# LeoQLi/DeepSIR

Measured on AMD Instinct MI355X. Metric: registered pairs/sec (5k-pt 3DMatch-shaped synthetic pairs, 5 registration iterations, KNN pyramid included), higher is better.
Workload: dtype f32 (GEMMs as fp16-pair MFMA, fp32 accumulate; index decisions exact fp32)

## Files before the change

deepsir_amd/_lib.py:

```python
from __future__ import annotations

import ctypes as C
import os

_HERE = os.path.dirname(os.path.abspath(__file__))
LIB_PATH = os.environ.get("DSIR_LIB", os.path.join(_HERE, "libdsir.so"))

c_float_p = C.POINTER(C.c_float)
c_i32_p = C.POINTER(C.c_int32)
c_i64_p = C.POINTER(C.c_int64)


class dsir_cfg(C.Structure):
    _fields_ = [
        ("feat_len", C.c_int32),
        ("num_knn", C.c_int32),
        ("num_layers", C.c_int32),
        ("sub_sampling_ratio", C.c_int32 * 4),
        ("d_out", C.c_int32 * 4),
        ("out_feat_dim", C.c_int32),
        ("num_classes", C.c_int32),
        ("max_points", C.c_int32),
        ("max_pairs", C.c_int32),
        ("pipeline", C.c_int32),
# ... 46 lines not shown
    "dsir_create_ex": (C.c_int, [C.c_int, C.POINTER(dsir_cfg), C.c_int, C.POINTER(C.c_void_p)]),
    "dsir_destroy": (None, [C.c_void_p]),
    "dsir_last_error": (C.c_char_p, [C.c_void_p]),
    "dsir_stream": (C.c_void_p, [C.c_void_p]),
    "dsir_sync": (C.c_int, [C.c_void_p]),
    "dsir_set_stream": (C.c_int, [C.c_void_p, C.c_void_p, C.c_int]),
    "dsir_num_weights": (C.c_int, [C.c_void_p]),
    "dsir_weight_name": (C.c_char_p, [C.c_void_p, C.c_int, c_i64_p]),
    "dsir_load_weight": (C.c_int, [C.c_void_p, C.c_char_p, C.c_void_p, c_i64_p, C.c_int]),
    "dsir_finalize_weights": (C.c_int, [C.c_void_p]),
    "dsir_narrow_i64": (C.c_int, [C.c_void_p, C.c_void_p, C.c_void_p, C.c_int64]),
    "dsir_knn_pyramid": (C.c_int, [C.c_void_p, C.c_void_p, C.c_int, C.c_int, C.c_int, C.c_void_p, C.c_void_p,
                                   C.c_void_p, C.c_void_p]),
    "dsir_randla_forward": (C.c_int, [C.c_void_p, C.c_int, C.c_void_p, C.c_int, C.c_int, C.c_int, C.c_void_p,
                                      C.c_void_p, C.c_void_p, C.c_void_p, C.c_void_p, C.c_void_p]),
    "dsir_ppf_pre": (C.c_int, [C.c_void_p, C.c_int, C.c_void_p, C.c_int, C.c_void_p, C.c_int64, C.c_int, C.c_int, C.c_void_p]),
    "dsir_estimate_normals": (C.c_int, [C.c_void_p, C.c_void_p, C.c_int, C.c_void_p, C.c_int64, C.c_int, C.c_int, c_float_p, C.c_void_p,
                                        C.c_void_p]),
    "dsir_estimate_normals_csr": (C.c_int, [C.c_void_p, C.c_void_p, C.c_int, C.c_void_p, C.c_void_p, C.c_int, C.c_int, c_float_p, C.c_void_p,
                                            C.c_void_p]),
    "dsir_fpfh": (C.c_int, [C.c_void_p, C.c_void_p, C.c_int, C.c_void_p, C.c_void_p, C.c_int64, C.c_void_p, C.c_void_p, C.c_int, C.c_int,
                            C.c_void_p, C.c_int, C.c_void_p]),
    "dsir_iss_keypoints": (C.c_int, [C.c_void_p, C.c_void_p, C.c_int, C.c_void_p, C.c_void_p, C.c_void_p, C.c_void_p, C.c_int, C.c_int,
                                     C.c_double, C.c_double, C.c_int, C.c_void_p, C.c_void_p, C.c_void_p, C.c_void_p]),
    "dsir_score": (C.c_int, [C.c_void_p, C.c_void_p, C.c_void_p, C.c_void_p, C.c_int64, C.c_void_p, C.c_int64,
                             C.c_int, C.c_int, C.c_void_p, C.c_void_p]),
    "dsir_aggregate": (C.c_int, [C.c_void_p, C.c_void_p, C.c_int64, C.c_void_p, C.c_void_p, C.c_int, C.c_int,
                                 C.c_void_p]),
    "dsir_nn_match": (C.c_int, [C.c_void_p, C.c_void_p, C.c_void_p, C.c_int, C.c_int, C.c_int, C.c_void_p]),
    "dsir_nn_match_screened": (C.c_int, [C.c_void_p, C.c_void_p, C.c_void_p, C.c_int, C.c_int, C.c_int, C.c_void_p, c_i64_p]),
# ... 189 lines not shown
```

deepsir_amd/csrc/att_pool.hip:

```cpp
#include "kernels.h"
#include "device_utils.h"
#include "att_pool_body.h"

namespace dsir {

namespace {

using namespace attp;

template <bool UV>
__global__ __launch_bounds__(256) __attribute__((amdgpu_waves_per_eu(UV ? 4 : 5, UV ? 4 : 5))) void att_pool16_kernel(const AttPool16Args p) {
  constexpr int LD = 20;
  constexpr int TB = 32 * LD + 32;
  __shared__ float s_sc[16];
  __shared__ float s_sh[16];
  __shared__ __attribute__((aligned(16))) float s_t[4][TB + 32 * LD];

  const int tid = threadIdx.x, lane = tid & 63, w = __builtin_amdgcn_readfirstlane(tid >> 6);
  const int m = lane & 31, h = lane >> 5;
  const int wi = xcd_contiguous(blockIdx.x, gridDim.x);
  const int bx = wi % p.grid_x;
  const int cloud = wi / p.grid_x;

  float sc[8], sh[8];
  const float slope = (h ? p.enc_act : p.f_act) ? 0.2f : 1.f;

  h8 whA, wlA, whB, wlB;
  {
    const _Float16* Wh = reinterpret_cast<const _Float16*>(p.Wh);
    const _Float16* Wl = reinterpret_cast<const _Float16*>(p.Wl);
    const int col = m & 15;
// ... 2 lines not shown
    h8 z;
#pragma unroll
    for (int j = 0; j < 8; ++j) z[j] = (_Float16)0.f;
    whA = m < 16 ? vh : z; wlA = m < 16 ? vl : z;
    whB = m < 16 ? z : vh; wlB = m < 16 ? z : vl;
  }
  const int pm = (m >> 2) & 1, km = ((m >> 3) << 2) | (m & 3);
  const float* fb = p.f + cloud * p.f_cs;
  const float* eb = p.enc + cloud * p.enc_cs;
  const int32_t* nbb = p.neigh + cloud * p.neigh_cs;
  float* Yb = p.Y + cloud * p.y_cs;
  float* T = &s_t[w][0];
  const int etile = m >> 4, ecol = m & 15;

  const int units = (p.n + 3) >> 2;
  const int nw = p.grid_x * 4;
  int u = bx * 4 + w;

  auto point_of = [&](int uu, int tile) { return min(4 * uu + 2 * tile + pm, p.n - 1); };
  auto load_idx = [&](int uu, int (&j)[2]) {
#pragma unroll
    for (int t = 0; t < 2; ++t) j[t] = nbb[(uint32_t)point_of(uu, t) * 16u + (uint32_t)km];
  };
  const float* uvb = UV ? p.uv + cloud * p.uv_cs : nullptr;
  const float* distb = UV ? p.dist + cloud * p.dist_cs : nullptr;
  float wa[8];
#pragma unroll
  for (int c = 0; c < 8; ++c) wa[c] = UV ? p.w8[c * 8] : 0.f;
  auto load_rows = [&](int uu, const int (&j)[2], float (&a)[2][8], float (&v)[2][8], float (&dd)[2]) {
#pragma unroll
    for (int t = 0; t < 2; ++t) {
      const int pt = point_of(uu, t);
// ... 72 lines not shown
    float mx = fmaxf(acc[0], acc[1]);
#pragma unroll
    for (int i = 2; i < 16; i += 2) mx = fmaxf(mx, fmaxf(acc[i], acc[i + 1]));
    const float ml = -mx * L2E;
    float se = 0.f, o = 0.f;
    const float* Tc = &T[etile * TB + 4 * h * LD + ecol];
#pragma unroll
    for (int i = 0; i < 16; ++i) {
      const float e = __builtin_amdgcn_exp2f(fmaf(acc[i], L2E, ml));
      const float x = Tc[(8 * (i >> 2) + (i & 3)) * LD];
      se += e;
      o = fmaf(x, e, o);
    }
    const int pt = 4 * u + 2 * etile + h;
    if (pt < p.n) Yb[(uint32_t)pt * 16u + (uint32_t)ecol] = o * __builtin_amdgcn_rcpf(se);
    __builtin_amdgcn_wave_barrier();
#pragma unroll
    for (int t = 0; t < 2; ++t) {
#pragma unroll
      for (int j = 0; j < 8; ++j) { a[t][j] = an[t][j]; av[t][j] = avn[t][j]; }
      ad[t] = adn[t];
    }
    u = un;
  }
}

template <int KH, bool UV>
__global__ __launch_bounds__(256) __attribute__((amdgpu_waves_per_eu(KH == 32 ? 3 : 2, KH == 32 ? 3 : 2))) void att_full_kernel(const AttPool16Args p) {
  constexpr int NCB = KH / 32;
  __shared__ __attribute__((aligned(16))) char smem[att_full_smem_bytes<KH>()];
  const int wi = xcd_contiguous(blockIdx.x, gridDim.x);
  att_full_body<KH, UV>(p, wi % p.grid_x, (wi / p.grid_x) % NCB, wi / (p.grid_x * NCB), smem);
}

__global__ __launch_bounds__(512) void att_full128_kernel(const AttPool16Args p) {
  constexpr int KH = 64, KC = 64, NS = 8, NT = 4;
  constexpr int LD = 72;
  __shared__ float s_sc[2 * KH];
// ... 125 lines not shown
          const float e = __builtin_amdgcn_exp2f(fmaf(acc[tt][i], L2E, ml));
          const float x = Tc[(8 * (i >> 2) + (i & 3)) * LD];
          se += e;
          o = fmaf(x, e, o);
        }
        if (pt < p.n) Yb[(uint32_t)pt * (uint32_t)(2 * KH) + (uint32_t)(64 * tp + 32 * tt + m)] = o * __builtin_amdgcn_rcpf(se);
      }
      __builtin_amdgcn_wave_barrier();
    }
    u = un;
  }
}

}

bool launch_att_pool16(const AttPool16Args& a, hipStream_t st) {
  if (a.n <= 0 || a.clouds <= 0) return true;
  if (!a.Wh || !a.Wl || !a.f || !a.neigh || !a.Y) return false;
  if (!a.enc && (!a.uv || !a.dist || !a.w8 || (reinterpret_cast<uintptr_t>(a.uv) % 16) != 0 || (a.uv_cs % 4) != 0)) return false;
  if ((a.ldw % 8) != 0 || (reinterpret_cast<uintptr_t>(a.Wh) % 16) != 0 || (reinterpret_cast<uintptr_t>(a.Wl) % 16) != 0) return false;
  if ((reinterpret_cast<uintptr_t>(a.f) % 16) != 0 || (a.f_cs % 4) != 0 || (a.f_ld % 4) != 0 || (a.enc && ((reinterpret_cast<uintptr_t>(a.enc) % 16) != 0 || (a.enc_cs % 4) != 0))) return false;
  if ((a.f_gn.stats && (8 % a.f_gn.groups) != 0) || (a.enc_gn.stats && (8 % a.enc_gn.groups) != 0)) return false;
  if ((int64_t)a.n * 16 * 8 * 4 >= ((int64_t)1 << 32)) return false;
  const int units = (a.n + 3) / 4;
  int blocks = (units + 31) / 32;
  const int64_t total = (int64_t)blocks * a.clouds;
  if (total < 512) {
    const int want = (int)((512 + (int64_t)a.clouds - 1) / (int64_t)a.clouds), most = (units + 3) / 4;
    const int nb = want < most ? want : most;
    if (nb > blocks) blocks = nb;
  }
  if (blocks < 1) blocks = 1;
  AttPool16Args b = a;
  b.grid_x = blocks;
  if (a.enc) hipLaunchKernelGGL(att_pool16_kernel<false>, dim3((unsigned)((int64_t)blocks * a.clouds)), dim3(256), 0, st, b);
  else hipLaunchKernelGGL(att_pool16_kernel<true>, dim3((unsigned)((int64_t)blocks * a.clouds)), dim3(256), 0, st, b);
  return true;
}

bool launch_att_full(const AttPool16Args& a, int KH, hipStream_t st) {
  if (a.n <= 0 || a.clouds <= 0) return true;
  if ((KH != 32 && KH != 64) || !a.Wh || !a.Wl || !a.f || !a.neigh || !a.Y) return false;
  if (!a.enc && (KH != 32 || !a.uv || !a.dist || !a.w8 || (reinterpret_cast<uintptr_t>(a.uv) % 16) != 0 || (a.uv_cs % 4) != 0)) return false;
  if ((a.ldw % 8) != 0 || (reinterpret_cast<uintptr_t>(a.Wh) % 16) != 0 || (reinterpret_cast<uintptr_t>(a.Wl) % 16) != 0) return false;
  if ((reinterpret_cast<uintptr_t>(a.f) % 16) != 0 || (a.f_cs % 4) != 0 || (a.f_ld % 4) != 0 || (a.enc && ((reinterpret_cast<uintptr_t>(a.enc) % 16) != 0 || (a.enc_cs % 4) != 0))) return false;
  if ((a.f_gn.stats && (KH % a.f_gn.groups) != 0) || (a.enc_gn.stats && (KH % a.enc_gn.groups) != 0)) return false;
  if ((int64_t)a.n * 16 * KH * 4 >= ((int64_t)1 << 32)) return false;
  const int units = (a.n + 1) / 2;
  if (KH == 64 && (int64_t)units * a.clouds >= 8192) {
    int blocks = (units + 63) / 64;
    if ((int64_t)blocks * a.clouds < 256) {
      const int want = (int)((256 + (int64_t)a.clouds - 1) / (int64_t)a.clouds), most = (units + 7) / 8;
      const int nb = want < most ? want : most;
      if (nb > blocks) blocks = nb;
    }
    if (blocks < 1) blocks = 1;
// ... 41 lines not shown
```

deepsir_amd/csrc/device_utils.h:

```cpp
#pragma once
#include <hip/hip_runtime.h>
#include <stdint.h>

namespace dsir {

typedef float f32x4 __attribute__((ext_vector_type(4)));

#ifndef DSIR_GN_WORDS_DEFINED
#define DSIR_GN_WORDS_DEFINED
constexpr int kGnWords = 4;
#endif

__device__ __forceinline__ float ld_f32(const float* base, uint32_t byte_off) {
  return *reinterpret_cast<const float*>(reinterpret_cast<const char*>(base) + byte_off);
}
__device__ __forceinline__ int ld_i32(const int32_t* base, uint32_t byte_off) {
  return *reinterpret_cast<const int32_t*>(reinterpret_cast<const char*>(base) + byte_off);
}
__device__ __forceinline__ void st_f32(float* base, uint32_t byte_off, float v) {
  *reinterpret_cast<float*>(reinterpret_cast<char*>(base) + byte_off) = v;
}

__device__ __forceinline__ int xcd_contiguous(int id, int nwg) {
  const int q8 = nwg >> 3, r8 = nwg & 7, xcd = id & 7;
// ... 62 lines not shown
  return v;
}

__device__ __forceinline__ float se3_row(const float* T, int r, float x, float y, float z) {
  return __fadd_rn(fmaf(z, T[r * 4 + 2], fmaf(y, T[r * 4 + 1], __fmul_rn(x, T[r * 4 + 0]))), T[r * 4 + 3]);
}

__device__ __forceinline__ float exp_neg(float x) {
  return __builtin_amdgcn_exp2f(x * 1.44269504088896340736f);
}

__device__ __forceinline__ double gn_stat_limb(double v, int limb) {
  const double l1 = rint(v * 0x1p-24);
  return limb ? rint(fma(-l1, 0x1p24, v) * 0x1p16) : l1;
}
__device__ __forceinline__ void gn_block_commit(const float* part, int n0, int ncols, int gw, double* stats_cloud) {
  const int g0 = n0 / gw, ng = (n0 + ncols - 1) / gw - g0 + 1;
  const int t = threadIdx.x, j = t & 15;
  for (int q = t >> 4; q < ((ng * 2 + 15) & ~15); q += 16) {
    const bool live = q < ng * 2;
    const int g = g0 + (q >> 1), stat = q & 1;
    const int c0 = max(g * gw, n0) - n0, c1 = min((g + 1) * gw, n0 + ncols) - n0;
    double d = 0.0;
    if (live)
      for (int c = c0 + j; c < c1; c += 16) d += (double)part[c * 2 + stat];
    d += __shfl_xor(d, 1); d += __shfl_xor(d, 2); d += __shfl_xor(d, 4); d += __shfl_xor(d, 8);
    if (live && j < 2)
      unsafeAtomicAdd(stats_cloud + (int64_t)g * kGnWords + 2 * stat + j, gn_stat_limb(d, j));
  }
}
__device__ __forceinline__ double gn_rstd(double var) {
  const double v = var + 1e-5;
  double r = __builtin_amdgcn_rsq(v);
  r = fma(r, fma(-0.5 * v * r, r, 0.5), r);
  r = fma(r, fma(-0.5 * v * r, r, 0.5), r);
  return r;
}
__device__ __forceinline__ double gn_stat_get(const double* slot) {
#ifdef DSIR_GN_STATS_COHERENT
  const double l1 = __hip_atomic_load(slot, __ATOMIC_RELAXED, __HIP_MEMORY_SCOPE_AGENT);
  const double l0 = __hip_atomic_load(slot + 1, __ATOMIC_RELAXED, __HIP_MEMORY_SCOPE_AGENT);
  return fma(l1, 0x1p24, l0 * 0x1p-16);
#else
  return fma(slot[0], 0x1p24, slot[1] * 0x1p-16);
// ... 64 lines not shown
```

deepsir_amd/csrc/engine_ctx.h:

```cpp
#pragma once
#include <hip/hip_runtime.h>

#include <string>
#include <unordered_map>
#include <vector>

#include "dsir.h"
#include "kernels.h"
#include "search_plan.h"

namespace dsir {

struct HostParam {
  std::string name;
  std::vector<int64_t> shape;
  std::vector<float> data;
  bool loaded = false;
  bool ignored = false;
  int64_t numel() const { int64_t n = 1; for (auto s : shape) n *= s; return n; }
};

struct Mlp2dW { const float *W = nullptr, *b = nullptr, *gamma = nullptr, *beta = nullptr; int cin = 0, cout = 0, groups = 0; };
struct AttW { const float* fc = nullptr; const float* fc_g = nullptr; int d = 0; Mlp2dW mlp; };
struct BlockW { Mlp2dW mlp1, lfa1, lfa2, mlp2, skip; AttW att1, att2; int d_in = 0, d = 0; const float* lse_w8 = nullptr;
// ... 183 lines not shown
  float* dist_buf[DSIR_MAX_LEVELS] = {};
  float* enc2_buf[DSIR_MAX_LEVELS] = {};
  double* enc_stats[DSIR_MAX_LEVELS] = {};
  double* enc2_stats[DSIR_MAX_LEVELS] = {};
  Act enc[DSIR_MAX_LEVELS], enc2[DSIR_MAX_LEVELS];
  static size_t stats_words(const dsir_cfg& g, int P) { return (size_t)2 * g.num_layers * gn_layer_words(P); }
  int plan(dsir_ctx* c, const Pyramid& ps, double* prezeroed);
};

struct AggExtras { float* sq = nullptr; void* hi = nullptr; void* lo = nullptr; unsigned long long* packed_init = nullptr; };

void fill_pyramid_layout(const dsir_cfg& cfg, int clouds, int n, Pyramid& p);
int gn_max_contributions(const dsir_cfg& g, int n, int flags = 0);
int randla_forward(dsir_ctx* c, const RandlaW& w, const Seg& in0, const Seg* in1, const Pyramid& py, float* feat_out,
                   float* logits_out, EncCache* cache = nullptr);
int run_ppf_pre(dsir_ctx* c, const RandlaW& w, const float* rows, int stride, const int32_t* neigh, int64_t neigh_cs, int clouds, int n,
                float* out);
float* run_mlp_feat(dsir_ctx* c, const float* feat0, int clouds, int n, float* out = nullptr);
bool run_att_proj(dsir_ctx* c, const float* xyz, int64_t xyz_cs, const float* score, const float* F, int clouds, int n,
                  float* desc, const AggExtras* ex = nullptr);
int build_pyramid(dsir_ctx* c, const float* points, int stride, int clouds, int n, float* xyz, int32_t* neigh,
                  int32_t* sub, int32_t* interp);

void expect_state_dict(dsir_ctx* c);

struct DescSearch {
  dsir_ctx* c;
  SearchMode mode;
  int P, J, K;
  bool timed = false;
// ... 33 lines not shown
```

deepsir_amd/csrc/entries_stage.hip:

```cpp
#include <cmath>

#include "engine_ctx.h"

using namespace dsir;

extern "C" {

int dsir_narrow_i64(dsir_ctx* c, const int64_t* src, int32_t* dst, int64_t n) {
  Call call(c); if (call.refused()) return 1;
  launch_narrow_i64(src, dst, n, c->stream);
  return call.finish();
}

int dsir_knn_pyramid(dsir_ctx* c, const float* points, int stride, int clouds, int n, float* xyz, int32_t* neigh,
                     int32_t* sub, int32_t* interp) {
  Call call(c); if (call.refused()) return 1;
  if (clouds < 1 || stride < 3) return fail(c, "dsir_knn_pyramid: bad arguments");
  if (int r = build_pyramid(c, points, stride, clouds, n, xyz, neigh, sub, interp)) return r;
  return call.finish();
}

int dsir_randla_forward(dsir_ctx* c, int which, const float* features, int cin, int clouds, int n, const float* xyz,
                        const int32_t* neigh, const int32_t* sub, const int32_t* interp, float* feat, float* logits) {
  Call call(c, Call::kWeights); if (call.refused()) return 1;
  if (which != 0 && c->cfg.pipeline != DSIR_PIPELINE_ALIGN) return fail(c, "randla_forward: this context has no inlier_model (pipeline != align)");
  const RandlaW& w = which == 0 ? c->net.feat : c->net.inl;
  if (w.ppf ? cin < 6 : cin != w.cin)
    return w.ppf ? fail(c, "randla_forward: use_ppf needs rows of xyz + normal, at least 6 columns, got %d (reference RandLANet.py:325)", cin)
                 : fail(c, "randla_forward: expected %d input channels, got %d", w.cin, cin);
  if (check_batch(c, "randla_forward", clouds, n)) return 1;
  Pyramid py;
  fill_pyramid_layout(c->cfg, clouds, n, py);
  if (py.nl[3] < kKnn) return fail(c, "cloud too small (n=%d)", n);
  py.xyz = xyz; py.neigh = neigh; py.sub = sub; py.interp = interp;
  const Seg in0 = plain_seg(features, (int64_t)n * cin, w.ppf ? 3 : cin, cin);
  const Seg in1 = plain_seg(features + 3, (int64_t)n * cin, 3, cin);
  if (int r = call.begin_walker()) return r;
  if (int r = randla_forward(c, w, in0, w.ppf ? &in1 : nullptr, py, feat, logits)) return r;
  return call.finish();
}

int dsir_ppf_pre(dsir_ctx* c, int which, const float* rows, int stride, const int32_t* neigh, int64_t neigh_cs, int clouds, int n,
                 float* out) {
  Call call(c, Call::kWeights); if (call.refused()) return 1;
  if (!(c->flags & DSIR_FLAG_PPF)) return fail(c, "dsir_ppf_pre: the context was not created with DSIR_FLAG_PPF");
  if (which != 0 && c->cfg.pipeline != DSIR_PIPELINE_ALIGN) return fail(c, "dsir_ppf_pre: this context has no inlier_model (pipeline != align)");
  if (!rows || !neigh || !out || clouds < 1 || n < kKnn) return fail(c, "dsir_ppf_pre: bad arguments");
  if (stride < 6) return fail(c, "dsir_ppf_pre: rows of xyz + normal need at least 6 columns, got %d (reference RandLANet.py:325)", stride);
  if (check_batch(c, "dsir_ppf_pre", clouds, n)) return 1;
  if (int r = run_ppf_pre(c, which == 0 ? c->net.feat : c->net.inl, rows, stride, neigh, neigh_cs, clouds, n, out)) return r;
  return call.finish();
}

// ... 128 lines not shown
```

deepsir_amd/csrc/kernels.h:

```cpp
#pragma once
#include <hip/hip_runtime.h>
#include <stdint.h>
#include <stdlib.h>

namespace dsir {

constexpr int kKnn = 16;

const char* tuning_env(const char* name);
inline bool tuning_flag(const char* name) { return tuning_env(name) != nullptr; }
inline long long tuning_int(const char* name, long long dflt) { const char* e = tuning_env(name); return e ? atoll(e) : dflt; }

#ifndef DSIR_GN_WORDS_DEFINED
#define DSIR_GN_WORDS_DEFINED
constexpr int kGnWords = 4;
#endif
struct GnRef {
  const double* stats;
  const float* gamma;
  const float* beta;
  int groups;
  double inv_count;
};

// ... 78 lines not shown
  const float* enc = nullptr;
  int64_t enc_cs = 0;
  const float* uv = nullptr; int64_t uv_cs = 0;
  const float* dist = nullptr; int64_t dist_cs = 0;
  const float* w8 = nullptr;
  GnRef enc_gn = {nullptr, nullptr, nullptr, 0, 0.0}; int enc_act = 1;
  const int32_t* neigh = nullptr;
  int64_t neigh_cs = 0;
  const void* Wh = nullptr;
  const void* Wl = nullptr;
  int ldw = 16;
  float* Y = nullptr;
  int64_t y_cs = 0;
  int n = 0, clouds = 0;
  int grid_x = 0;
};
bool launch_att_pool16(const AttPool16Args& a, hipStream_t st);
bool launch_att_full(const AttPool16Args& a, int KH, hipStream_t st);

struct LseUvArgs {
  const float* xyz = nullptr; int64_t xyz_cs = 0;
  const int32_t* neigh = nullptr; int64_t neigh_cs = 0;
  const float* w8 = nullptr;
  float* uv = nullptr; int64_t uv_cs = 0;
  float* dist = nullptr; int64_t dist_cs = 0;
  double* stats_out = nullptr; int groups = 0;
  int n = 0, clouds = 0, KH = 0;
  int vgrid = 0;
};
bool launch_lse_uv_stats(const LseUvArgs& a, hipStream_t st);

struct PpfArgs {
// ... 340 lines not shown
```

deepsir_amd/csrc/schedule.hip:

```cpp
#include <cstddef>
#include <cstring>
#include <vector>

#include "engine_ctx.h"

namespace dsir {

namespace {
void level_sizes(const dsir_cfg& cfg, int n, int* nl) {
  nl[0] = n;
  for (int l = 0; l < cfg.num_layers; ++l) nl[l + 1] = nl[l] / cfg.sub_sampling_ratio[l];
}
}

void fill_pyramid_layout(const dsir_cfg& cfg, int clouds, int n, Pyramid& p) {
  p.clouds = clouds; p.n = n;
  level_sizes(cfg, n, p.nl);
  p.off[0] = 0; p.soff[0] = 0;
  for (int l = 0; l < cfg.num_layers; ++l) { p.off[l + 1] = p.off[l] + p.nl[l]; p.soff[l + 1] = p.soff[l] + p.nl[l + 1]; }
  p.S = p.off[cfg.num_layers]; p.S1 = p.soff[cfg.num_layers];
}

int gn_max_contributions(const dsir_cfg& g, int n, int flags) {
  const bool ppf = (flags & DSIR_FLAG_PPF) != 0;
// ... 2 lines not shown
    const int groups = cout >= 64 ? 8 : 4;
    const int c = cin <= 64 ? pw_stream_gn_contributions(M, cout) : pw_tile_gn_contributions(M, cout, groups);
    if (c > worst) worst = c;
  };
  int nl[DSIR_MAX_LEVELS + 1];
  level_sizes(g, n, nl);
  const int L = g.num_layers;
  if (ppf) { const int c = ppf_gn_contributions(nl[0]); if (c > worst) worst = c; }
  else layer(nl[0], 6 > g.feat_len ? 6 : g.feat_len, 8);
  int dim = ppf ? 12 : 8;
  for (int l = 0; l < L; ++l) {
    const int d = g.d_out[l], m = nl[l], mk = nl[l] * kKnn;
    if (ppf && l == 0) { const int c = pw_gemm_gn_contributions(m); if (c > worst) worst = c; }
    else { layer(m, dim, d / 2); layer(m, dim, 2 * d); }
    if (d / 2 == 8 || d / 2 == 32) { const int c = lse_uv_gn_contributions(m, d / 2); if (c > worst) worst = c; }
    layer(mk, 10, d / 2);
    layer(mk, d / 2, d / 2);
    layer(m, d, d / 2); layer(m, d, d); layer(m, d, 2 * d);
    dim = 2 * d;
  }
  layer(nl[L], dim, dim);
  int dcur = dim;
  for (int j = 0; j < L; ++j) {
    const int lvl = L - 1 - j;
    const int cin = j < L - 1 ? dcur + 2 * g.d_out[L - j - 2] : 4 * g.d_out[0];
    dcur = j < L - 1 ? 2 * g.d_out[L - j - 2] : 2 * g.d_out[0];
    layer(nl[lvl], cin, dcur);
  }
  return worst;
}
// ... 177 lines not shown
    rec_flush();
    if (!c->ws.overflow && !launch_pw_gemm(a, st)) refuse("lfa.mlp1: no kernel took the relative-position layer");
    return y;
  }
  AttPool16Args att_pool_args(const AttW& w, const Act& f, const Act& enc, const int32_t* neigh, int64_t neigh_cs, int n, const Act& y) const {
    AttPool16Args a;
    a.f = f.p; a.f_cs = (int64_t)f.rows * f.C; a.f_ld = f.C; a.f_gn = f.gn; a.f_act = f.act;
    a.enc = enc.p; a.enc_cs = (int64_t)enc.rows * enc.C; a.enc_gn = enc.gn; a.enc_act = enc.act;
    a.uv = enc.uv; a.uv_cs = (int64_t)n * 2 * enc.C; a.dist = enc.dist; a.dist_cs = (int64_t)n * kKnn; a.w8 = enc.w8;
    a.neigh = neigh; a.neigh_cs = neigh_cs;
    const size_t off = (size_t)(w.fc - c->dweights);
    a.Wh = c->dweights16 + off; a.Wl = c->dweights16 + c->nweights + off; a.ldw = w.d;
    a.Y = y.p; a.y_cs = (int64_t)n * w.d; a.n = n; a.clouds = clouds;
    return a;
  }
  Act att(const AttW& w, const Act& f, const Act& enc, const int32_t* neigh, int64_t neigh_cs, int n, float* s2 = nullptr,
          int s2_mode = 0) {
    Act y;
    y.p = c->ws.get<float>((size_t)clouds * n * w.d);
    y.C = w.d; y.rows = n;
    const bool halves = f.C * 2 == w.d && enc.C * 2 == w.d;
    const bool fc16 = c->dweights16 && w.fc >= c->dweights && w.fc < c->dweights + c->nweights;
    if (w.d == 16 && halves && fc16) {
      const AttPool16Args a = att_pool_args(w, f, enc, neigh, neigh_cs, n, y);
      rec_flush();
      if (!c->ws.overflow && launch_att_pool16(a, st)) return y;
    } else if ((w.d == 64 || w.d == 128) && halves && fc16 && (enc.p || w.d == 64)) {
      const AttPool16Args a = att_pool_args(w, f, enc, neigh, neigh_cs, n, y);
      if (c->ws.overflow) return y;
      if (rec) {
        WalkJob j;
        if (walk_plan_att_full(a, w.d / 2, rec_wpc, &j) && rec_push(j)) return y;
        rec_flush();
      }
      if (launch_att_full(a, w.d / 2, st)) return y;
    } else if (att_keeps_score_cache(w.d) && w.fc_g && halves && enc.p) {
      float* G = c->ws.get<float>((size_t)clouds * n * w.d);
      GemmArgs g;
      g.amode = A_SEGS; g.nseg = 1; g.seg[0] = seg_of(f);
      g.W = w.fc_g; g.ldw = w.d / 2; g.bias = nullptr; g.Cin = w.d / 2; g.Cout = w.d; g.M = n; g.clouds = clouds;
// ... 93 lines not shown
  for (int l = 0; l < g.num_layers; ++l) {
    enc_stats[l] = cst + (size_t)(2 * l) * gn_layer_words(P);
    enc2_stats[l] = cst + (size_t)(2 * l + 1) * gn_layer_words(P);
  }
  return 0;
}

int run_ppf_pre(dsir_ctx* c, const RandlaW& w, const float* rows, int stride, const int32_t* neigh, int64_t neigh_cs, int clouds, int n,
                float* out) {
  const size_t stats_need = gn_layer_words(clouds, 4);
  if (stats_need > c->stats_cap) return fail(c, "stats arena too small (%zu > %zu)", stats_need, c->stats_cap);
  c->call.stats_top = 0;
  HIP_OK(c, hipMemsetAsync(c->stats, 0, stats_need * sizeof(double), c->stream));
  Sched s{c, c->stream, clouds};
  s.ppf_pre(w.pre, plain_seg(rows, (int64_t)n * stride, 3, stride), plain_seg(rows + 3, (int64_t)n * stride, 3, stride), neigh, neigh_cs, n, out);
  return 0;
}

int randla_forward(dsir_ctx* c, const RandlaW& w, const Seg& in0, const Seg* in1, const Pyramid& py, float* feat_out,
                   float* logits_out, EncCache* cache) {
  const dsir_cfg& g = c->cfg;
  const int L = g.num_layers;
  hipStream_t st = c->stream;
  Sched s{c, st, py.clouds};
  const size_t stats_need = gn_pass_words(py.clouds);
  if (c->call.stats_prezeroed && c->call.stats_base + stats_need <= c->stats_cap) {
    c->call.stats_top = c->call.stats_base;
    c->call.stats_base += stats_need;
  } else {
    c->call.stats_top = 0;
// ... 33 lines not shown
  Act enc_pre[DSIR_MAX_LEVELS], enc2_pre[DSIR_MAX_LEVELS];
  if (w.ppf && !in1) return fail(c, "randla_forward: the point-pair-feature layer needs normals");
  Act x = w.ppf ? s.ppf_pre(w.pre, in0, *in1, py.neigh, neigh_cs, py.nl[0]) : s.mlp2d(w.pre, in0, in1, py.nl[0], true);
  std::vector<Act> skips;
  for (int l = 0; l < L; ++l) {
    const BlockW& b = w.blk[l];
    const int n = py.nl[l];
    const int32_t* nb_l = py.neigh + (int64_t)py.off[l] * kKnn;
    const Seg xin = Sched::seg_of(x);
    Act f, skipb;
    const bool ahead = walk && l >= walk_from;
    const bool paired = s.mlp2d_pair(b, xin, n, f, skipb);
    if (!paired) f = s.mlp2d(b.mlp1, xin, nullptr, n, true);
    const Act enc = ahead ? enc_pre[l] : enc_of(l);
    const int s2_mode = reuse ? 2 : 1;
    Act agg = s.att(b.att1, f, enc, nb_l, neigh_cs, n, cache ? cache->s2_buf[l][0] : nullptr, s2_mode);
    Act a1 = s.mlp2d(b.att1.mlp, Sched::seg_of(agg), nullptr, n, true);
    const Act enc2 = ahead ? enc2_pre[l] : enc2_of(l, enc);
    if (cache && !reuse) { cache->enc[l] = enc; cache->enc2[l] = enc2; }
    Act agg2 = s.att(b.att2, a1, enc2, nb_l, neigh_cs, n, cache ? cache->s2_buf[l][1] : nullptr, s2_mode);
    Act a2 = s.mlp2d(b.att2.mlp, Sched::seg_of(agg2), nullptr, n, true);
    Act mainb = s.mlp2d(b.mlp2, Sched::seg_of(a2), nullptr, n, false);
    if (!paired) skipb = s.mlp2d(b.skip, xin, nullptr, n, false);
    Act enc_out;
    enc_out.C = 2 * b.d; enc_out.rows = n;
    Act samp;
    samp.C = enc_out.C; samp.rows = py.nl[l + 1];
    samp.p = c->ws.get<float>((size_t)py.clouds * samp.rows * samp.C);
    if (l == 0) enc_out.p = c->ws.get<float>((size_t)py.clouds * n * enc_out.C);
    if (c->ws.overflow) {
      if (c->call.sched_error) return fail(c, "randla_forward: %s (level %d)", c->call.sched_error, l);
      return fail(c, "workspace exhausted in randla_forward (raise max_points / max_pairs)");
    }
// ... 175 lines not shown
```

deepsir_amd/engine.py:

```python
from __future__ import annotations

import ctypes as C
from typing import Dict, Optional, Sequence, Tuple

import numpy as np
import torch

from . import _lib
from .arch import PIPELINES, NetConfig, level_sizes


class EngineError(RuntimeError):
    pass


def check_pose_weight(w) -> float:
    w = float(w)
    if not (w >= 0.0) or w == float("inf"):
        raise EngineError(f"align_loss_backward: wt_pose_loss must be finite and >= 0, got {w}")
    return w


def _ptr(t: Optional[torch.Tensor]) -> Optional[int]:
    return None if t is None else t.data_ptr()
# ... 160 lines not shown

    def randla_forward(self, which: str, features, xyz, neigh, sub, interp, want_logits=True):
        features = _chk(features, torch.float32, "features")
        c, n, cin = features.shape
        w = {"feat_extractor": 0, "inlier_model": 1}[which]
        ncls = self.cfg.num_classes if w == 0 else 1
        feat = self._empty((c, n, 64))
        logits = self._empty((c, n, ncls)) if want_logits else None
        xyz, neigh, sub, interp = (_chk(xyz, torch.float32, "xyz"), _chk(neigh, torch.int32, "neigh_idx"),
                                   _chk(sub, torch.int32, "sub_idx"), _chk(interp, torch.int32, "interp_idx"))
        self._pre()
        self._call(self.lib.dsir_randla_forward(self.h, w, _ptr(features), cin, c, n, _ptr(xyz), _ptr(neigh), _ptr(sub),
                                                _ptr(interp), _ptr(feat), _ptr(logits)))
        self.sync()
        return feat, logits

    def ppf_pre(self, which: str, rows, neigh_multi):
        rows, neigh_multi = _chk(rows, torch.float32, "rows"), _chk(neigh_multi, torch.int32, "neigh_idx")
        c, n, stride = rows.shape
        out = self._empty((c, n, 12))
        self._pre()
        self._call(self.lib.dsir_ppf_pre(self.h, {"feat_extractor": 0, "inlier_model": 1}[which], _ptr(rows), stride, _ptr(neigh_multi),
                                         neigh_multi.shape[1] * 16, c, n, _ptr(out)))
        self.sync()
        return out

    def estimate_normals(self, points, neigh_multi=None, viewpoint=(0.0, 0.0, 0.0), csr=None):
        points = _chk(points, torch.float32, "points")
        if (neigh_multi is None) == (csr is None):
            raise EngineError("estimate_normals: exactly one of neigh_multi and csr expected")
# ... 885 lines not shown
```

include/dsir.h:

```cpp
#ifndef DSIR_H
#define DSIR_H

#include <stdint.h>
#include <stddef.h>

#ifdef __cplusplus
extern "C" {
#endif

#define DSIR_MAX_LEVELS 4
#define DSIR_KNN 16

typedef struct dsir_ctx dsir_ctx;

typedef struct dsir_cfg {
  int32_t feat_len;
  int32_t num_knn;
  int32_t num_layers;
  int32_t sub_sampling_ratio[DSIR_MAX_LEVELS];
  int32_t d_out[DSIR_MAX_LEVELS];
  int32_t out_feat_dim;
  int32_t num_classes;
  int32_t max_points;
  int32_t max_pairs;
// ... 16 lines not shown
int dsir_num_weights(const dsir_ctx* ctx);
const char* dsir_weight_name(const dsir_ctx* ctx, int i, int64_t* numel);

int dsir_load_weight(dsir_ctx* ctx, const char* key, const float* host_data, const int64_t* shape, int ndim);
int dsir_finalize_weights(dsir_ctx* ctx);


int dsir_narrow_i64(dsir_ctx* ctx, const int64_t* src, int32_t* dst, int64_t n);

int dsir_knn_pyramid(dsir_ctx* ctx, const float* points, int stride, int clouds, int n,
                     float* xyz_multi, int32_t* neigh_idx, int32_t* sub_idx, int32_t* interp_idx);

int dsir_randla_forward(dsir_ctx* ctx, int which, const float* features, int cin, int clouds, int n,
                        const float* xyz_multi, const int32_t* neigh_idx, const int32_t* sub_idx,
                        const int32_t* interp_idx, float* feat, float* logits);

int dsir_ppf_pre(dsir_ctx* ctx, int which, const float* rows, int stride, const int32_t* neigh_idx, int64_t neigh_cloud_stride,
                 int clouds, int n, float* out);

int dsir_estimate_normals(dsir_ctx* ctx, const float* points, int stride, const int32_t* neigh_idx, int64_t neigh_cloud_stride,
                          int clouds, int n, const float* viewpoint, float* normals, int32_t* flags);
int dsir_estimate_normals_csr(dsir_ctx* ctx, const float* points, int stride, const int32_t* csr_offsets, const int32_t* csr_cols,
                              int clouds, int n, const float* viewpoint, float* normals, int32_t* flags);

int dsir_fpfh(dsir_ctx* ctx, const float* points, int stride, const float* normals, const int32_t* neigh_idx,
              int64_t neigh_cloud_stride, const int32_t* csr_offsets, const int32_t* csr_cols, int clouds, int n, float* desc,
              int out_ld, int32_t* flags);

int dsir_iss_keypoints(dsir_ctx* ctx, const float* points, int stride, const int32_t* sal_offsets, const int32_t* sal_cols,
                       const int32_t* nms_offsets, const int32_t* nms_cols, int clouds, int n, double gamma_21, double gamma_32,
// ... 233 lines not shown
```

Before: 5187.

## Fuse lfa.mlp2 encoding GEMM and GroupNorm stats into first attentive pooling kernel

For d=16 levels with position-encoding tables, the first attentive-pooling kernel now also computes the second local-feature encoding (an 8x8 linear layer via MFMA on the rebuilt encoding rows held in shared memory). It writes those rows and commits GroupNorm partial statistics per wave, replacing a separate mlp2d pass over the enc tensor. This removes one kernel launch and a re-read of the encoding. In exchange, the grid is sized by the GN contribution count, extra LDS is used, and per-wave work grows. A gating threshold on block count plus an env flag control it, and a probe entry point is added for validation.

```diff
diff --git a/deepsir_amd/_lib.py b/deepsir_amd/_lib.py
--- a/deepsir_amd/_lib.py
+++ b/deepsir_amd/_lib.py
@@ -84,6 +84,7 @@
                                    C.c_void_p, C.c_void_p]),
     "dsir_randla_forward": (C.c_int, [C.c_void_p, C.c_int, C.c_void_p, C.c_int, C.c_int, C.c_int, C.c_void_p,
                                       C.c_void_p, C.c_void_p, C.c_void_p, C.c_void_p, C.c_void_p]),
+    "dsir_lfa_enc2_probe": (C.c_int, [C.c_void_p, C.c_int, C.c_int, C.c_int, C.c_int, C.c_int, C.c_void_p, C.c_void_p, C.c_void_p, C.c_void_p]),
     "dsir_ppf_pre": (C.c_int, [C.c_void_p, C.c_int, C.c_void_p, C.c_int, C.c_void_p, C.c_int64, C.c_int, C.c_int, C.c_void_p]),
     "dsir_estimate_normals": (C.c_int, [C.c_void_p, C.c_void_p, C.c_int, C.c_void_p, C.c_int64, C.c_int, C.c_int, c_float_p, C.c_void_p,
                                         C.c_void_p]),
diff --git a/deepsir_amd/csrc/att_pool.hip b/deepsir_amd/csrc/att_pool.hip
--- a/deepsir_amd/csrc/att_pool.hip
+++ b/deepsir_amd/csrc/att_pool.hip
@@ -8,13 +8,16 @@
 
 using namespace attp;
 
-template <bool UV>
+template <bool UV, bool E2 = false>
 __global__ __launch_bounds__(256) __attribute__((amdgpu_waves_per_eu(UV ? 4 : 5, UV ? 4 : 5))) void att_pool16_kernel(const AttPool16Args p) {
+  static_assert(UV || !E2, "the producing variant rebuilds E from the tables");
   constexpr int LD = 20;
   constexpr int TB = 32 * LD + 32;
   __shared__ float s_sc[16];
   __shared__ float s_sh[16];
   __shared__ __attribute__((aligned(16))) float s_t[4][TB + 32 * LD];
+  __shared__ float s_e2w[E2 ? 3 * 64 : 1];
+  __shared__ float s_g[E2 ? 4 * 8 * 64 : 1];
 
   const int tid = threadIdx.x, lane = tid & 63, w = __builtin_amdgcn_readfirstlane(tid >> 6);
   const int m = lane & 31, h = lane >> 5;
@@ -47,8 +50,21 @@
   const int etile = m >> 4, ecol = m & 15;
 
   const int units = (p.n + 3) >> 2;
-  const int nw = p.grid_x * 4;
-  int u = bx * 4 + w;
+  const int nw = E2 ? p.e2_vgx : p.grid_x * 4;
+  const int gwave = bx * 4 + w;
+  int u = (E2 && gwave >= nw) ? units : gwave;
+  const int fr = lane & 15, fq = lane >> 4;
+  float* G = &s_g[E2 ? w * 8 * 64 + lane : 0];
+  if (E2) {
+    if (w == 0) {
+      s_e2w[lane] = fr < 8 ? p.e2_W[fr * 8 + 2 * fq] : 0.f;
+      s_e2w[64 + lane] = fr < 8 ? p.e2_W[fr * 8 + 2 * fq + 1] : 0.f;
+      s_e2w[128 + lane] = (fr < 8 && p.e2_b) ? p.e2_b[fr] : 0.f;
+    }
+#pragma unroll
+    for (int q = 0; q < 8; ++q) G[q * 64] = 0.f;
+  }
+  float* E2b = E2 ? p.e2_Y + cloud * p.e2_cs : nullptr;
 
   auto point_of = [&](int uu, int tile) { return min(4 * uu + 2 * tile + pm, p.n - 1); };
   auto load_idx = [&](int uu, int (&j)[2]) {
@@ -151,6 +167,29 @@
     }
     const int pt = 4 * u + 2 * etile + h;
     if (pt < p.n) Yb[(uint32_t)pt * 16u + (uint32_t)ecol] = o * __builtin_amdgcn_rcpf(se);
+    if (E2) {
+#pragma unroll
+      for (int q = 0; q < 4; ++q) {
+        const int mr = ((fr >> 2) << 3) | ((q & 1) << 2) | (fr & 3);
+        const float2 ev = *reinterpret_cast<const float2*>(&T[(q >> 1) * TB + mr * LD + 8 + 2 * fq]);
+        f32x4 c = f32x4{0.f, 0.f, 0.f, 0.f};
+        c = __builtin_amdgcn_mfma_f32_16x16x4f32(ev.x, s_e2w[lane], c, 0, 0, 0);
+        c = __builtin_amdgcn_mfma_f32_16x16x4f32(ev.y, s_e2w[64 + lane], c, 0, 0, 0);
+        const int pq = 4 * u + q;
+        if (pq < p.n && fr < 8) {
+          const float e2b = s_e2w[128 + lane];
+          float g1 = G[(2 * q) * 64], g2 = G[(2 * q + 1) * 64];
+#pragma unroll
+          for (int r = 0; r < 4; ++r) {
+            const float v = c[r] + e2b;
+            st_f32(E2b, 4u * ((uint32_t)(pq * 16 + 4 * fq + r) * 8u + (uint32_t)fr), v);
+            g1 += v;
+            g2 += v * v;
+          }
+          G[(2 * q) * 64] = g1; G[(2 * q + 1) * 64] = g2;
+        }
+      }
+    }
     __builtin_amdgcn_wave_barrier();
 #pragma unroll
     for (int t = 0; t < 2; ++t) {
@@ -159,6 +198,19 @@
       ad[t] = adn[t];
     }
     u = un;
+  }
+  if (E2 && gwave < nw) {
+    float c1 = 0.f, c2 = 0.f;
+#pragma unroll
+    for (int q = 0; q < 4; ++q) {
+      float s1 = G[(2 * q) * 64], s2 = G[(2 * q + 1) * 64];
+      s1 += __shfl_xor(s1, 16); s1 += __shfl_xor(s1, 32);
+      s2 += __shfl_xor(s2, 16); s2 += __shfl_xor(s2, 32);
+      c1 += s1; c2 += s2;
+    }
+    if (lane < 16) { T[lane * 2] = c1; T[lane * 2 + 1] = c2; }
+    __builtin_amdgcn_wave_barrier();
+    gn_wave_commit(T, 0, 8, 8 / p.e2_groups, p.e2_stats + (int64_t)cloud * p.e2_groups * kGnWords);
   }
 }
 
@@ -314,8 +366,16 @@
 
 }
 
+bool att_pool16_produces(const AttPool16Args& a) {
+  if (!a.e2_W || a.enc || !a.uv || a.n <= 0) return false;
+  if (a.e2_groups < 1 || (8 % a.e2_groups) != 0) return false;
+  return att_pool16_gn_contributions(a.n) <= kGnMaxContrib;
+}
+int att_pool16_gn_contributions(int n) { return pw_stream_gn_contributions(n * 16, 8); }
+
 bool launch_att_pool16(const AttPool16Args& a, hipStream_t st) {
   if (a.n <= 0 || a.clouds <= 0) return true;
+  if ((a.e2_Y || a.e2_W) && (!a.e2_Y || !a.e2_stats || !att_pool16_produces(a))) return false;
   if (!a.Wh || !a.Wl || !a.f || !a.neigh || !a.Y) return false;
   if (!a.enc && (!a.uv || !a.dist || !a.w8 || (reinterpret_cast<uintptr_t>(a.uv) % 16) != 0 || (a.uv_cs % 4) != 0)) return false;
   if ((a.ldw % 8) != 0 || (reinterpret_cast<uintptr_t>(a.Wh) % 16) != 0 || (reinterpret_cast<uintptr_t>(a.Wl) % 16) != 0) return false;
@@ -332,6 +392,13 @@
   }
   if (blocks < 1) blocks = 1;
   AttPool16Args b = a;
+  if (a.e2_Y) {
+    b.e2_vgx = att_pool16_gn_contributions(a.n);
+    blocks = (b.e2_vgx + 3) / 4;
+    b.grid_x = blocks;
+    hipLaunchKernelGGL((att_pool16_kernel<true, true>), dim3((unsigned)((int64_t)blocks * a.clouds)), dim3(256), 0, st, b);
+    return true;
+  }
   b.grid_x = blocks;
   if (a.enc) hipLaunchKernelGGL(att_pool16_kernel<false>, dim3((unsigned)((int64_t)blocks * a.clouds)), dim3(256), 0, st, b);
   else hipLaunchKernelGGL(att_pool16_kernel<true>, dim3((unsigned)((int64_t)blocks * a.clouds)), dim3(256), 0, st, b);
@@ -340,6 +407,7 @@
 
 bool launch_att_full(const AttPool16Args& a, int KH, hipStream_t st) {
   if (a.n <= 0 || a.clouds <= 0) return true;
+  if (a.e2_Y || a.e2_W) return false;
   if ((KH != 32 && KH != 64) || !a.Wh || !a.Wl || !a.f || !a.neigh || !a.Y) return false;
   if (!a.enc && (KH != 32 || !a.uv || !a.dist || !a.w8 || (reinterpret_cast<uintptr_t>(a.uv) % 16) != 0 || (a.uv_cs % 4) != 0)) return false;
   if ((a.ldw % 8) != 0 || (reinterpret_cast<uintptr_t>(a.Wh) % 16) != 0 || (reinterpret_cast<uintptr_t>(a.Wl) % 16) != 0) return false;
diff --git a/deepsir_amd/csrc/device_utils.h b/deepsir_amd/csrc/device_utils.h
--- a/deepsir_amd/csrc/device_utils.h
+++ b/deepsir_amd/csrc/device_utils.h
@@ -100,10 +100,12 @@
   const double l1 = rint(v * 0x1p-24);
   return limb ? rint(fma(-l1, 0x1p24, v) * 0x1p16) : l1;
 }
+template <int NT = 256>
 __device__ __forceinline__ void gn_block_commit(const float* part, int n0, int ncols, int gw, double* stats_cloud) {
   const int g0 = n0 / gw, ng = (n0 + ncols - 1) / gw - g0 + 1;
-  const int t = threadIdx.x, j = t & 15;
-  for (int q = t >> 4; q < ((ng * 2 + 15) & ~15); q += 16) {
+  const int t = NT == 256 ? threadIdx.x : threadIdx.x & (NT - 1), j = t & 15;
+  constexpr int QT = NT / 16;
+  for (int q = t >> 4; q < ((ng * 2 + QT - 1) & ~(QT - 1)); q += QT) {
     const bool live = q < ng * 2;
     const int g = g0 + (q >> 1), stat = q & 1;
     const int c0 = max(g * gw, n0) - n0, c1 = min((g + 1) * gw, n0 + ncols) - n0;
@@ -114,6 +116,9 @@
     if (live && j < 2)
       unsafeAtomicAdd(stats_cloud + (int64_t)g * kGnWords + 2 * stat + j, gn_stat_limb(d, j));
   }
+}
+__device__ __forceinline__ void gn_wave_commit(const float* part, int n0, int ncols, int gw, double* stats_cloud) {
+  gn_block_commit<64>(part, n0, ncols, gw, stats_cloud);
 }
 __device__ __forceinline__ double gn_rstd(double var) {
   const double v = var + 1e-5;
diff --git a/deepsir_amd/csrc/engine_ctx.h b/deepsir_amd/csrc/engine_ctx.h
--- a/deepsir_amd/csrc/engine_ctx.h
+++ b/deepsir_amd/csrc/engine_ctx.h
@@ -221,6 +221,7 @@
 int gn_max_contributions(const dsir_cfg& g, int n, int flags = 0);
 int randla_forward(dsir_ctx* c, const RandlaW& w, const Seg& in0, const Seg* in1, const Pyramid& py, float* feat_out,
                    float* logits_out, EncCache* cache = nullptr);
+int run_lfa_enc2_probe(dsir_ctx* c, const RandlaW& w, int level, int fused, const Pyramid& py, float* rows_out, double* stats_out);
 int run_ppf_pre(dsir_ctx* c, const RandlaW& w, const float* rows, int stride, const int32_t* neigh, int64_t neigh_cs, int clouds, int n,
                 float* out);
 float* run_mlp_feat(dsir_ctx* c, const float* feat0, int clouds, int n, float* out = nullptr);
diff --git a/deepsir_amd/csrc/entries_stage.hip b/deepsir_amd/csrc/entries_stage.hip
--- a/deepsir_amd/csrc/entries_stage.hip
+++ b/deepsir_amd/csrc/entries_stage.hip
@@ -37,6 +37,20 @@
   const Seg in1 = plain_seg(features + 3, (int64_t)n * cin, 3, cin);
   if (int r = call.begin_walker()) return r;
   if (int r = randla_forward(c, w, in0, w.ppf ? &in1 : nullptr, py, feat, logits)) return r;
+  return call.finish();
+}
+
+int dsir_lfa_enc2_probe(dsir_ctx* c, int which, int level, int fused, int clouds, int n, const float* xyz, const int32_t* neigh,
+                        float* rows, double* stats) {
+  Call call(c, Call::kWeights); if (call.refused()) return 1;
+  if (which != 0 && c->cfg.pipeline != DSIR_PIPELINE_ALIGN) return fail(c, "dsir_lfa_enc2_probe: this context has no inlier_model (pipeline != align)");
+  if (!xyz || !neigh || !rows || !stats || clouds < 1 || level < 0 || level >= c->cfg.num_layers) return fail(c, "dsir_lfa_enc2_probe: bad arguments");
+  if (check_batch(c, "dsir_lfa_enc2_probe", clouds, n)) return 1;
+  Pyramid py;
+  fill_pyramid_layout(c->cfg, clouds, n, py);
+  if (py.nl[c->cfg.num_layers - 1] < kKnn) return fail(c, "cloud too small (n=%d)", n);
+  py.xyz = xyz; py.neigh = neigh;
+  if (int r = run_lfa_enc2_probe(c, which == 0 ? c->net.feat : c->net.inl, level, fused, py, rows, stats)) return r;
   return call.finish();
 }
 
diff --git a/deepsir_amd/csrc/kernels.h b/deepsir_amd/csrc/kernels.h
--- a/deepsir_amd/csrc/kernels.h
+++ b/deepsir_amd/csrc/kernels.h
@@ -116,8 +116,17 @@
   int64_t y_cs = 0;
   int n = 0, clouds = 0;
   int grid_x = 0;
+  const float* e2_W = nullptr;
+  const float* e2_b = nullptr;
+  float* e2_Y = nullptr;
+  int64_t e2_cs = 0;
+  double* e2_stats = nullptr;
+  int e2_groups = 0;
+  int e2_vgx = 0;
 };
 bool launch_att_pool16(const AttPool16Args& a, hipStream_t st);
+bool att_pool16_produces(const AttPool16Args& a);
+int att_pool16_gn_contributions(int n);
 bool launch_att_full(const AttPool16Args& a, int KH, hipStream_t st);
 
 struct LseUvArgs {
diff --git a/deepsir_amd/csrc/schedule.hip b/deepsir_amd/csrc/schedule.hip
--- a/deepsir_amd/csrc/schedule.hip
+++ b/deepsir_amd/csrc/schedule.hip
@@ -40,6 +40,7 @@
     if (ppf && l == 0) { const int c = pw_gemm_gn_contributions(m); if (c > worst) worst = c; }
     else { layer(m, dim, d / 2); layer(m, dim, 2 * d); }
     if (d / 2 == 8 || d / 2 == 32) { const int c = lse_uv_gn_contributions(m, d / 2); if (c > worst) worst = c; }
+    if (d / 2 == 8) { const int c = att_pool16_gn_contributions(m); if (c > worst) worst = c; }
     layer(mk, 10, d / 2);
     layer(mk, d / 2, d / 2);
     layer(m, d, d / 2); layer(m, d, d); layer(m, d, 2 * d);
@@ -247,16 +248,40 @@
     a.Y = y.p; a.y_cs = (int64_t)n * w.d; a.n = n; a.clouds = clouds;
     return a;
   }
+  struct AttEnc2 {
+    const Mlp2dW* w = nullptr;
+    float* buf = nullptr;
+    double* stats = nullptr;
+    bool done = false;
+    Act out;
+  };
   Act att(const AttW& w, const Act& f, const Act& enc, const int32_t* neigh, int64_t neigh_cs, int n, float* s2 = nullptr,
-          int s2_mode = 0) {
+          int s2_mode = 0, AttEnc2* e2 = nullptr) {
     Act y;
     y.p = c->ws.get<float>((size_t)clouds * n * w.d);
     y.C = w.d; y.rows = n;
     const bool halves = f.C * 2 == w.d && enc.C * 2 == w.d;
     const bool fc16 = c->dweights16 && w.fc >= c->dweights && w.fc < c->dweights + c->nweights;
     if (w.d == 16 && halves && fc16) {
-      const AttPool16Args a = att_pool_args(w, f, enc, neigh, neigh_cs, n, y);
+      AttPool16Args a = att_pool_args(w, f, enc, neigh, neigh_cs, n, y);
       rec_flush();
+      if (e2 && e2->w && enc.uv && !enc.p && e2->w->cin == 8 && e2->w->cout == 8) {
+        a.e2_W = e2->w->W; a.e2_b = e2->w->b; a.e2_groups = e2->w->groups;
+        if (att_pool16_produces(a)) {
+          const int M = n * kKnn;
+          Act& o = e2->out;
+          o.p = e2->buf ? e2->buf : c->ws.get<float>((size_t)clouds * M * 8);
+          o.C = 8; o.rows = M; o.act = 1;
+          double* st_out = e2->stats ? e2->stats : stats_slot(e2->w->groups);
+          o.gn = gn_of(st_out, *e2->w, M);
+          a.e2_Y = o.p; a.e2_cs = (int64_t)M * 8; a.e2_stats = st_out;
+          if (c->ws.overflow) return y;
+          if (launch_att_pool16(a, st)) { e2->done = true; return y; }
+          refuse("attentive pooling: the producing variant refused a layer it had accepted");
+          return y;
+        }
+        a.e2_W = a.e2_b = nullptr; a.e2_groups = 0;
+      }
       if (!c->ws.overflow && launch_att_pool16(a, st)) return y;
     } else if ((w.d == 64 || w.d == 128) && halves && fc16 && (enc.p || w.d == 64)) {
       const AttPool16Args a = att_pool_args(w, f, enc, neigh, neigh_cs, n, y);
@@ -380,6 +405,43 @@
   HIP_OK(c, hipMemsetAsync(c->stats, 0, stats_need * sizeof(double), c->stream));
   Sched s{c, c->stream, clouds};
   s.ppf_pre(w.pre, plain_seg(rows, (int64_t)n * stride, 3, stride), plain_seg(rows + 3, (int64_t)n * stride, 3, stride), neigh, neigh_cs, n, out);
+  return 0;
+}
+
+int run_lfa_enc2_probe(dsir_ctx* c, const RandlaW& w, int level, int fused, const Pyramid& py, float* rows_out, double* stats_out) {
+  const BlockW& b = w.blk[level];
+  if (!b.lse_w8 || !lse_uv_enabled()) return fail(c, "lfa_enc2_probe: level %d has no position-encoding tables", level);
+  const int n = py.nl[level], M = n * kKnn, ch = b.lfa2.cout;
+  hipStream_t st = c->stream;
+  const size_t stats_need = 2 * gn_layer_words(py.clouds);
+  if (stats_need > c->stats_cap) return fail(c, "stats arena too small (%zu > %zu)", stats_need, c->stats_cap);
+  c->call.stats_top = 0;
+  HIP_OK(c, hipMemsetAsync(c->stats, 0, stats_need * sizeof(double), st));
+  Sched s{c, st, py.clouds};
+  const int64_t xyz_cs = (int64_t)py.S * 3, neigh_cs = (int64_t)py.S * kKnn;
+  const int32_t* nb_l = py.neigh + (int64_t)py.off[level] * kKnn;
+  const Act enc = s.lse_uv(b.lfa1, b.lse_w8, py.xyz + (int64_t)py.off[level] * 3, xyz_cs, nb_l, neigh_cs, n, nullptr, nullptr, nullptr);
+  Act enc2;
+  if (fused) {
+    Act f;
+    f.C = b.d / 2; f.rows = n; f.act = 1;
+    f.p = c->ws.get<float>((size_t)py.clouds * n * f.C);
+    if (c->ws.overflow) return overflow_fail(c, "workspace exhausted in lfa_enc2_probe");
+    HIP_OK(c, hipMemsetAsync(f.p, 0, sizeof(float) * py.clouds * n * f.C, st));
+    Sched::AttEnc2 e2;
+    e2.w = &b.lfa2;
+    s.att(b.att1, f, enc, nb_l, neigh_cs, n, nullptr, 0, &e2);
+    if (!c->ws.overflow && !e2.done) return fail(c, "lfa_enc2_probe: the first pooling of level %d does not produce lfa.mlp2", level);
+    enc2 = e2.out;
+  } else {
+    enc2 = s.mlp2d(b.lfa2, Sched::seg_of(enc, nb_l, neigh_cs), nullptr, M, true);
+  }
+  if (c->ws.overflow) {
+    if (c->call.sched_error) return fail(c, "lfa_enc2_probe: %s (level %d)", c->call.sched_error, level);
+    return overflow_fail(c, "workspace exhausted in lfa_enc2_probe");
+  }
+  HIP_OK(c, hipMemcpyAsync(rows_out, enc2.p, sizeof(float) * py.clouds * M * ch, hipMemcpyDeviceToDevice, st));
+  HIP_OK(c, hipMemcpyAsync(stats_out, enc2.gn.stats, sizeof(double) * py.clouds * b.lfa2.groups * kGnWords, hipMemcpyDeviceToDevice, st));
   return 0;
 }
 
@@ -443,9 +505,18 @@
     if (!paired) f = s.mlp2d(b.mlp1, xin, nullptr, n, true);
     const Act enc = ahead ? enc_pre[l] : enc_of(l);
     const int s2_mode = reuse ? 2 : 1;
-    Act agg = s.att(b.att1, f, enc, nb_l, neigh_cs, n, cache ? cache->s2_buf[l][0] : nullptr, s2_mode);
+    static const bool no_att_enc2 = tuning_flag("DSIR_NO_ATT_ENC2");
+    static const long long att_enc2_min = tuning_int("DSIR_ATT_ENC2_MIN_BLOCKS", 512);
+    Sched::AttEnc2 e2;
+    if (!no_att_enc2 && !reuse && !ahead && enc.uv && !enc.p && b.d == 16 &&
+        (int64_t)((att_pool16_gn_contributions(n) + 3) / 4) * py.clouds >= att_enc2_min) {
+      e2.w = &b.lfa2;
+      e2.buf = cache ? cache->enc2_buf[l] : nullptr;
+      e2.stats = cache ? cache->enc2_stats[l] : nullptr;
+    }
+    Act agg = s.att(b.att1, f, enc, nb_l, neigh_cs, n, cache ? cache->s2_buf[l][0] : nullptr, s2_mode, e2.w ? &e2 : nullptr);
     Act a1 = s.mlp2d(b.att1.mlp, Sched::seg_of(agg), nullptr, n, true);
-    const Act enc2 = ahead ? enc2_pre[l] : enc2_of(l, enc);
+    const Act enc2 = ahead ? enc2_pre[l] : (e2.done ? e2.out : enc2_of(l, enc));
     if (cache && !reuse) { cache->enc[l] = enc; cache->enc2[l] = enc2; }
     Act agg2 = s.att(b.att2, a1, enc2, nb_l, neigh_cs, n, cache ? cache->s2_buf[l][1] : nullptr, s2_mode);
     Act a2 = s.mlp2d(b.att2.mlp, Sched::seg_of(agg2), nullptr, n, true);
diff --git a/deepsir_amd/engine.py b/deepsir_amd/engine.py
--- a/deepsir_amd/engine.py
+++ b/deepsir_amd/engine.py
@@ -198,6 +198,22 @@
                                                 _ptr(interp), _ptr(feat), _ptr(logits)))
         self.sync()
         return feat, logits
+
+    def lfa_enc2_probe(self, which: str, level: int, fused: bool, xyz, neigh, n: int):
+        xyz, neigh = _chk(xyz, torch.float32, "xyz"), _chk(neigh, torch.int32, "neigh_idx")
+        c = xyz.shape[0]
+        assert xyz.shape[1] == self.pyramid_shapes(n)[0]
+        nl = n
+        for r in self.cfg.sub_sampling_ratio[:level]:
+            nl //= r
+        ch = self.cfg.d_out[level] // 2
+        rows = self._empty((c, 16 * nl, ch))
+        stats = self._empty((c, 8 if ch >= 64 else 4, 4), torch.float64)
+        self._pre()
+        self._call(self.lib.dsir_lfa_enc2_probe(self.h, {"feat_extractor": 0, "inlier_model": 1}[which], level, int(fused), c, n, _ptr(xyz),
+                                                _ptr(neigh), _ptr(rows), _ptr(stats)))
+        self.sync()
+        return rows, stats
 
     def ppf_pre(self, which: str, rows, neigh_multi):
         rows, neigh_multi = _chk(rows, torch.float32, "rows"), _chk(neigh_multi, torch.int32, "neigh_idx")
diff --git a/include/dsir.h b/include/dsir.h
--- a/include/dsir.h
+++ b/include/dsir.h
@@ -54,6 +54,9 @@
 int dsir_randla_forward(dsir_ctx* ctx, int which, const float* features, int cin, int clouds, int n,
                         const float* xyz_multi, const int32_t* neigh_idx, const int32_t* sub_idx,
                         const int32_t* interp_idx, float* feat, float* logits);
+
+int dsir_lfa_enc2_probe(dsir_ctx* ctx, int which, int level, int fused, int clouds, int n, const float* xyz_multi,
+                        const int32_t* neigh_idx, float* rows, double* stats);
 
 int dsir_ppf_pre(dsir_ctx* ctx, int which, const float* rows, int stride, const int32_t* neigh_idx, int64_t neigh_cloud_stride,
                  int clouds, int n, float* out);
```

Result: faster. 5250, median of 6 (+1.2%).
